# UNC-CFD/somar

Measured on AMD Instinct MI355X. Metric: pressure-Poisson V-cycles/sec, higher is better.
Workload: dtype f64; 1 GPU; C2 single-level 512^3 Poisson, diagonal stretched metric, Neumann, LevelGSRB V-cycle 2/2/2 + BiCGStab bottom; layout = 1 box(es) 512x512x512, one per GPU; mg_depth=8, cells=134217728

## Files before the change

somar_amd/build.py:

```python
import os
import subprocess
import sys

HERE = os.path.dirname(os.path.abspath(__file__))
CSRC = os.path.join(HERE, "csrc")
OUT = os.path.join(HERE, "libsomar_amd.so")
SOURCES = ["kernels.hip", "box_bicgstab.hip", "gsrb_fused.hip", "resid_march.hip", "multi_march.hip", "full19.hip", "full19_march.hip", "full19_fused.hip", "projection.hip", "line_gsrb.hip", "amr_kernels.hip", "leptic_kernels.hip", "maps.hip", "metric_refresh.hip", "box_io.hip", "tuning.cpp", "level.cpp", "solver.cpp", "solver_full.cpp", "solver_multi.cpp", "amr.cpp", "leptic.cpp", "comm_rccl.cpp", "comm_shm.cpp", "capi.cpp"]
HEADERS = ["common.h", "devbuf.h", "tuning.h", "kernels.h", "level.h", "march_plan.h", "stencil_point.h", "solver.h", "amr.h", "leptic.h", os.path.join("..", "..", "include", "somar_amd.h")]
HIPCC = os.environ.get("HIPCC", "/opt/rocm/bin/hipcc")
FLAGS = ["--offload-arch=gfx950", "-O3", "-std=c++17", "-fPIC", "-ffp-contract=off", "-fno-fast-math",
         "-Wall", "-Wno-unused-result", "-Wno-unused-value", "-I/opt/rocm/include"]


EXTRA = os.environ.get("SOMAR_EXTRA_FLAGS", "").split()


def _stale():
    if not os.path.exists(OUT):
        return True
    t = os.path.getmtime(OUT)
    return any(os.path.getmtime(os.path.join(CSRC, f)) > t for f in SOURCES + HEADERS)


def build(force=False, verbose=False):
    if not (force or _stale()):
        return OUT
    objs = []
    for f in SOURCES:
        src = os.path.join(CSRC, f)
        obj = os.path.join(CSRC, os.path.splitext(f)[0] + ".o")
        cmd = [HIPCC] + FLAGS + EXTRA + (["-x", "hip"] if f.endswith(".cpp") else []) + ["-c", src, "-o", obj]
        if verbose:
            print(" ".join(cmd))
        subprocess.check_call(cmd)
        objs.append(obj)
    cmd = [HIPCC, "--offload-arch=gfx950", "-shared", "-fPIC", "-o", OUT] + objs + ["-ldl", "-lrt"]
    if verbose:
        print(" ".join(cmd))
    subprocess.check_call(cmd)
    return OUT


if __name__ == "__main__":
    print(build(force="--force" in sys.argv, verbose=True))
```

somar_amd/csrc/kernels.h:

```cpp
#pragma once
#include "common.h"

namespace somar {

struct TileSpan {
    const Tile* p = nullptr;
    int n = 0;
    int classes = 0;
};

struct LevelDev {
    const Tile* tiles = nullptr;
    int ntiles = 0;
    int tile_j = 4;
    const CopyItem* tile_items = nullptr;
    const int* tile_item_start = nullptr;
    int ghost_gy = 16;
    const PatchDesc* patches = nullptr;
    int npatches = 0;
    double* jg[3] = {nullptr, nullptr, nullptr};
    double* jinv = nullptr;
    double* lapdiag = nullptr;
    double* jgf[3][3] = {{nullptr, nullptr, nullptr}, {nullptr, nullptr, nullptr}, {nullptr, nullptr, nullptr}};
    StencilParams P;
// ... 97 lines not shown
void launch_convert(hipStream_t st, float* dst, const double* src, long long n, double scale = 1.0);
void launch_incr2(hipStream_t st, double* y1, const double* x1, double a1, double* y2, const double* x2, double a2, long long n);
void launch_bicg_p(hipStream_t st, double* p, const double* v, const double* r, double beta, double bw, long long n);
void launch_incr_copy(hipStream_t st, double* y, double* x, double a, long long n);
void launch_scale(hipStream_t st, double* y, double a, long long n);
void launch_mul(hipStream_t st, double* y, const double* x, long long n);
void launch_axby(hipStream_t st, double* z, const double* x, const double* y, double a, double b, long long n);
struct ScalarPublish { double* host_dst; unsigned long long* host_seq; unsigned long long seq; };
struct TinyBicg {
    const Tile* tiles; int ntiles; int tile_j;
    const PatchDesc* patches; int npatches;
    const CopyItem* items; int nitems;
    long long field_elems;
    const double* jg[3]; const double* jinv; const double* lapd;
    StencilParams P;
    double* phi; const double* rhs;
    double* w[8];
    int imax, numRestarts, normType, precondIters;
    double eps, reps, hang, small, metric;
    double* info;
    ScalarPublish pub;
};
void launch_tiny_bicgstab(hipStream_t st, const LevelDev& L, const CopyItem* items, int nitems, long long field_elems, TinyBicg A);
constexpr int BOX_MAX_WG = 128, BOX_MAX_CELLS = 2048;
constexpr int BOX_FAB_MAX = 2048, BOX_MAX_ENT = 2048, BOX_MAX_STAGES = 63, BOX_MAX_NEUM = 512;
struct alignas(4) BoxProgEntry {
    unsigned short dst, s1, s2, s3;
    unsigned char kind, flags;
    unsigned short nslot;
};
struct BoxBicg {
    const PatchDesc* patches; int npatches;
    const int* nb; const int* cstart;
    const double* jg[3]; const double* jinv; const double* lapd;
    StencilParams P;
    double* phi; const double* rhs;
    double* z[2];
    int imax, numRestarts, normType, precondIters;
    double eps, reps, hang, small, metric;
    double* sums;
    unsigned* sync;
    int full;
    const double* jgf[3][3];
    const int* fab_src; const int* fab_start;
    const BoxProgEntry* ent[2]; const int* ent_first[2];
    const int* stg[2]; const int* stg_first[2];
    const int* nfg[2]; const int* nfg_first[2];
    long long* dbg;
    int serial;
    double* info;
    ScalarPublish pub;
};
void launch_box_bicgstab(hipStream_t st, const LevelDev& L, int max_box_cells, BoxBicg A);
void launch_stream_probe(hipStream_t st, int kind, int workgroups, double* const* in6, double* out, long long cells);
constexpr int MM_CH = 64;
struct CoarsenItem { const double* fine; double* crse; int patch; int dir; };
void launch_coarsen_metric(hipStream_t st, const LevelDev& C, const LevelDev& F, const CoarsenItem* items, int nitems,
                           int gy, const int r[3]);
struct MinMaxItem { const double* a; const PatchDesc* patches; int patch; int dir; };
void launch_minmax_all(hipStream_t st, const MinMaxItem* items, int nitems, double* out);
void launch_reduce(hipStream_t st, const LevelDev& L, const double* a, const double* b, int mode, double* partials,
                   double* out, bool ordered = false, const ScalarPublish* pub = nullptr);
void launch_reduce(hipStream_t st, const LevelDev& L, const float* a, const double* b, int mode, double* partials,
                   double* out);
void launch_ord_fill(hipStream_t st, const LevelDev& L, const long long* start, const double* a, const double* b,
                     int mode, double dxProduct, double* X, double* Y);
void launch_reduce_ordered_flat(hipStream_t st, int nboxes, const long long* box_start, const double* X, const double* Y,
                                int mode, double* out);
void launch_div_mac(hipStream_t st, const LevelDev& L, double* out, const double* u0, const double* u1,
                    const double* u2, double dt);
void launch_jgup_from_dxdxi(hipStream_t st, long long n, int mu, const double* const x9[9], const double* J, double scale,
                            double* out);
void launch_altered_jgup(hipStream_t st, long long n, double* dest, const double* nsq, const double* dmu,
                         const double* dnu, const double* ix, const double* jy, const double* iy, const double* jx,
                         const double* gup, const double* J, double theta, double coriolisF, bool offdiag);
void launch_face_axpy(hipStream_t st, const LevelDev& L, double* const vel[3], double* const grad[3], double s);
void launch_mac_correct(hipStream_t st, const LevelDev& L, double* const vel[3], const double* phi, double dtScale);
void launch_face_wall(hipStream_t st, const LevelDev& L, double* const edge[3]);
void launch_map_metric(hipStream_t st, const LevelDev& L, int kind, const double dXi[3], const double Lc[3],
                       const double* d_depth, const int dlo[2], const int dn[2], bool diagonal, const double* domLen = nullptr);
void launch_face_bc(hipStream_t st, const LevelDev& L, double* const edge[3], const int kind[6], const double value[6]);
void launch_cell_to_edge(hipStream_t st, const LevelDev& L, double* const edge[3], double* const cc[3], bool wall);
void launch_cc_correct(hipStream_t st, const LevelDev& L, double* const cc[3], const double* phi, double dtScale);
void launch_edge_to_cell_axpy(hipStream_t st, const LevelDev& L, double* const cc[3], double* const grad[3], double dtScale);
void launch_cf_homog(hipStream_t st, const CFCell* cells, int n, double* phi, const double c1[3], const double c2[3],
                     const double fac[3]);
void launch_copy_items2(hipStream_t st, const PatchDesc* spatches, const PatchDesc* dpatches, const CopyItem* items,
                        int nitems, const double* src, double* dst);
void launch_fill_hash(hipStream_t st, const LevelDev& L, double* f, unsigned long long seed);
constexpr int BIO_THREADS = 256, BIO_KC = 8;
struct BoxIoItem {
    int clo[3];
    int cpj;
    long long cpk;
    long long coff;
    int rlo[3];
    int n[3];
    int patch;
    int comp;
    int slot;
    int tile0, tiles_ij;
    int pad_;
};
void launch_box_io(hipStream_t st, const LevelDev& L, const BoxIoItem* items, double* const* ptrs, int nitems, int ntiles,
                   double* const field[3], bool to_level);

// ... 2 lines not shown
```

somar_amd/csrc/solver.cpp:

```cpp
#include "solver.h"

#include <array>
#include <chrono>
#include <cmath>
#include <cstdio>
#include <cstdlib>
#include <cstring>

namespace somar {

static const int S_MAX_COARSE = 4;
enum { SLOT_TMP = 0, SLOT_SUMS = 8, NSLOTS = 16 };

PressureSolver::PressureSolver(Comm* comm, hipStream_t shared, const Tuning& tune) : tune_(tune), comm_(comm ? comm : &self_)
{
    if (shared) { st_ = shared; own_stream_ = false; }
    else SOMAR_HIP(hipStreamCreateWithFlags(&st_, hipStreamNonBlocking));
    d_scalars = DevBuf<double>::zeros(NSLOTS);
    SOMAR_HIP(hipDeviceSynchronize());
    SOMAR_HIP(hipHostMalloc(&h_scalars, (NSLOTS + 2) * sizeof(double), hipHostMallocCoherent | hipHostMallocMapped));
    h_seq_ = reinterpret_cast<unsigned long long*>(h_scalars + NSLOTS);
    *h_seq_ = 0;
}

PressureSolver::~PressureSolver()
{
    drop_graphs();
    mp_free();
    mc_free();
    if (st_) hipStreamSynchronize(st_);
    if (st_comm_) { hipStreamSynchronize(st_comm_); hipStreamDestroy(st_comm_); }
    if (ev_ready_) hipEventDestroy(ev_ready_);
    if (ev_done_) hipEventDestroy(ev_done_);
    for (Prof& p : prof_) {
        for (hipEvent_t e : p.a) hipEventDestroy(e);
        for (hipEvent_t e : p.b) hipEventDestroy(e);
    }
    if (h_scalars) hipHostFree(h_scalars);
    coarse_.reset();
    lev.clear();
    if (st_ && own_stream_) hipStreamDestroy(st_);
}

void PressureSolver::sync() { SOMAR_HIP(hipStreamSynchronize(st_)); }

void PressureSolver::profile_enable(bool on)
{
    const int POOL = 4096;
    if (on)
        for (Prof& p : prof_) {
            while ((int)p.a.size() < POOL) {
                hipEvent_t e0, e1;
// ... 222 lines not shown
    std::unique_ptr<Level> C(new Level);
    C->active[2] = F.active[2];
    C->alpha = F.alpha;
    C->beta = F.beta;
    std::vector<IBox> cb;
    for (const IBox& b : F.boxes) cb.push_back(b.coarsen(r));
    double cdx[3];
    for (int d = 0; d < 3; ++d) cdx[d] = F.dx[d] * (double)r[d];
    C->define(F.domain.coarsen(r), F.periodic, cdx, F.bc_type, cb, F.owner, comm_, tune_);
    C->alloc_metric();
    if (hasCF_) C->define_cf(dxCrse_);
    for (int pi = 0; pi < C->npatches(); ++pi)
        for (int d = 0; d < nd; ++d)
            launch_avg_face(st_, C->dev, F.dev, pi, C->hpatches[pi].n, C->dev.jg[d], F.dev.jg[d], d, r);
    if (full_) {
        C->alloc_cross_metric();
        for (int pi = 0; pi < C->npatches(); ++pi)
            for (int d = 0; d < nd; ++d)
                for (int c = 0; c < nd; ++c)
                    if (c != d)
                        launch_avg_face(st_, C->dev, F.dev, pi, C->hpatches[pi].n, C->dev.jgf[d][c], F.dev.jgf[d][c], d, r);
    }
    launch_avg_harmonic(st_, C->dev, F.dev, C->dev.jinv, F.dev.jinv, r);
    launch_lapdiag(st_, C->dev);
    fill_metric_ghosts(*C);
    lev.push_back(std::move(C));
    return true;
}

void PressureSolver::fill_metric_ghosts(Level& L)
{
    for (int d = 0; d < 3; ++d)
        if (L.cf_faces[d]) L.cf_faces[d]->run(L.dev.jg[d], L.dev.jg[d], st_);
    for (int d = 0; d < 3; ++d) xchg(L, L.dev.jg[d]);
    if (full_)
        for (int d = 0; d < 3; ++d)
            for (int c = 0; c < 3; ++c)
                if (c != d && L.dev.jgf[d][c]) xchg(L, L.dev.jgf[d][c]);
    xchg(L, L.dev.jinv);
}

void PressureSolver::probe_null_space(int d)
{
    Level& L = *lev[d];
    DevBuf<double> phi = L.alloc_field(), rhs0 = L.alloc_field(), res = L.alloc_field();
    launch_set(st_, phi, L.field_elems, 0.0);
    apply_op(d, rhs0, phi);
    launch_set(st_, phi, L.field_elems, 1.0);
    residual(d, res, phi, rhs0);
    launch_reduce(st_, L.dev, res, nullptr, 3, d_partials, d_scalars + SLOT_TMP);
    comm_->allreduce(d_scalars + SLOT_TMP, 1, 1, st_);
    const double maxNorm = std::fabs(fetch_scalar(SLOT_TMP));
    L.zeroAvg = maxNorm < 0.01 * (probe_eps > 0.0 ? probe_eps : prm.eps);
}

void PressureSolver::finalize()
{
    SOMAR_CHECK(!lev.empty() && !finalized, "finalize before define / twice");
    if (mp_mode_ == 1) {
        const std::string why = mixed_refusal();
        SOMAR_CHECK(why.empty(), "finalize: mixed precision (set_precision mode 1) is not available for " + why);
    }
    const bool timing = tune_.timing != 0;
    auto now = [&]() { if (timing) hipDeviceSynchronize(); return std::chrono::steady_clock::now(); };
    auto secs = [](std::chrono::steady_clock::time_point a, std::chrono::steady_clock::time_point b) {
        return std::chrono::duration<double>(b - a).count();
    };
    const auto t0 = now();
    launch_lapdiag(st_, lev[0]->dev);
    fill_metric_ghosts(*lev[0]);
    int depth = 1;
    while (build_coarser(depth)) {
        if (comm_->size > 1 && lev[depth]->valid_cells_global <= tune_.agglom_cells && !full_) {
            build_agglomerated_tail(depth);
            break;
        }
        ++depth;
    }
    const auto t1 = now();
    detect_metric_flags();
    {
        const int min_box = (int)tune_.fused19_min_box;
        fused19_.assign(lev.size(), 0);
        for (size_t d = 0; d < lev.size(); ++d) {
            Level& L = *lev[d];
            bool ok = full_ && min_box >= 0 && full_march((int)d) && tune_.full_rows == 8 && !L.boxes.empty();
            for (const IBox& b : L.boxes)
                for (int a = 0; a < 3; ++a) ok = ok && b.size(a) >= std::max(min_box, 8) && (a != 0 || b.size(a) % 2 == 0);
            fused19_[d] = ok ? 1 : 0;
            if (ok != L.march.fused19) L.build_march_tiles(MarchRequest{L.march.narrow7, L.march.tall7, ok});
        }
    }
    choose_narrow_tiles();
    const auto t2 = now();
    struct Report {
        bool on; std::chrono::steady_clock::time_point t0, t1, t2; long long cells;
        ~Report() {
            if (!on) return;
            hipDeviceSynchronize();
            const auto t3 = std::chrono::steady_clock::now();
            fprintf(stderr, "[somar timing] finalize %lld cells: coarse hierarchy %.3f s, uniform detection %.3f s, fields + probes %.3f s\n",
                    cells, std::chrono::duration<double>(t1 - t0).count(), std::chrono::duration<double>(t2 - t1).count(),
                    std::chrono::duration<double>(t3 - t2).count());
        }
    } report{timing, t0, t1, t2, lev[0]->valid_cells_global};
    (void)secs;
// ... 1049 lines not shown
        double* eb[3] = {e[0], e[1], prm.spaceDim == 3 ? e[2] : nullptr};
        launch_face_bc(st_, lev[0]->dev, eb, velbc_kind_, velbc_value_);
    }
    divergence_mac(out, dt);
}

void PressureSolver::cc_correct(double* phi, double dt)
{
    Level& L = *lev[0];
    xchg(L, phi);
    double* c[3] = {cc_vel(0), cc_vel(1), prm.spaceDim == 3 ? cc_vel(2) : nullptr};
    const double dtScale = dt == 0.0 ? -1.0 : -dt;
    if (full_) {
        mac_grad_full(phi);
        launch_edge_to_cell_axpy(st_, L.dev, c, f_flux, dtScale);
        return;
    }
    launch_cc_correct(st_, L.dev, c, phi, dtScale);
}

void PressureSolver::cc_project(double dt, bool zeroPressure, bool forceHomogeneous, bool wall, SolveStats& s)
{
    check_idle("cc_project");
    divergence_cc(f_rhs, dt, wall);
    solve(zeroPressure, forceHomogeneous, s);
    cc_correct(f_phi, dt);
    sync();
}

void PressureSolver::fill_hash(int d, double* f, unsigned long long seed)
{
    launch_fill_hash(st_, lev[d]->dev, f, seed);
}

void PressureSolver::vcycle(double* e, const double* res, bool e_zero)
{
    check_idle("vcycle");
    if (mp_K_ > 0) {
        double rnorm = norm(0, res, 0);
        if (!e_zero) rnorm = std::max(rnorm, norm(0, e, 0));
        vcycle_mixed(e, res, rnorm, e_zero, false);
        return;
    }
    cycle(0, e, res, e_zero);
}

void PressureSolver::cycle_bottom_relax(double* corr, const double* res, bool corr_zero)
{
    const int d = (int)lev.size() - 1;
    if (lev[d]->domain.numPts() == 1) {
        relax(d, corr, res, 1, corr_zero);
        return;
    }
    if (corr_zero && prm.num_smooth_bottom == 0) launch_set(st_, corr, lev[d]->field_elems, 0.0);
    relax(d, corr, res, prm.num_smooth_bottom, corr_zero && prm.num_smooth_bottom > 0);
}

void PressureSolver::cycle_down(int d, double* corr, const double* res, bool corr_zero)
{
    if (corr_zero && prm.num_smooth_down == 0) launch_set(st_, corr, lev[d]->field_elems, 0.0);
    relax(d, corr, res, prm.num_smooth_down, corr_zero && prm.num_smooth_down > 0);
    restrict_residual(d, f_res[d + 1], corr, res);
}

void PressureSolver::cycle_up(int d, double* corr, const double* res)
{
    if (fold_prolong(d)) {
        fold_up(d, corr, res, f_corr[d + 1].get(), true);
        return;
    }
    const double* shift = prolong_increment(d, corr, f_corr[d + 1], fused_relax(d, prm.num_smooth_up));
    relax(d, corr, res, prm.num_smooth_up, false, shift);
}

void PressureSolver::cycle(int d, double* corr, const double* res, bool corr_zero)
{
    if (coarse_ && d == agglom_depth_) {
        agglom_cycle(corr, res, corr_zero);
        return;
    }
    const int D = (int)lev.size();
    if (mini_depth_ > 0 && d == mini_depth_ - 1) {
        (void)corr_zero;
        launch_set(st_, corr, lev[d]->field_elems, 0.0);
        return;
    }
    if (d == D - 1) {
        cycle_bottom_relax(corr, res, corr_zero);
        if (lev[d]->domain.numPts() != 1) bottom_solve(corr, res);
        return;
    }
    const int ncyc = cycle_override_ ? cycle_override_ : prm.numMG;
    SOMAR_CHECK(ncyc != 0, "numMG must not be 0");
    if (ncyc < 0) {
        const int cycles = -ncyc;
        Level& L = *lev[d];
        if (corr_zero) launch_set(st_, corr, L.field_elems, 0.0);
        restrict_residual(d, f_res[d + 1], corr, res);
        cycle(d + 1, f_corr[d + 1], f_res[d + 1], true);
        prolong_increment(d, corr, f_corr[d + 1]);
        relax(d, corr, res, prm.num_smooth_down);
        for (int img = 0; img < cycles; ++img) {
            restrict_residual(d, f_res[d + 1], corr, res);
            const int saved = cycle_override_;
            cycle_override_ = 1;
            try {
                cycle(d + 1, f_corr[d + 1], f_res[d + 1], true);
            } catch (...) {
                cycle_override_ = saved;
                throw;
            }
            cycle_override_ = saved;
            prolong_increment(d, corr, f_corr[d + 1]);
        }
        relax(d, corr, res, prm.num_smooth_up);
        return;
    }
    if (mini_depth_ == 0 && graph_cycle(d, corr, res, corr_zero)) return;
    cycle_down(d, corr, res, corr_zero);
// ... 820 lines not shown
```

somar_amd/csrc/solver.h:

```cpp
#pragma once
#include <exception>
#include <memory>
#include <vector>

#include "level.h"

namespace somar {

enum { RELAX_JACOBI = 0, RELAX_LEVEL_GSRB = 1, RELAX_LOOSE_GSRB = 2, RELAX_LINE_GSRB = 3 };
enum { PRECOND_NONE = -1, PRECOND_DIAG_RELAX = 0, PRECOND_DIAG_LINE_RELAX = 1 };

struct SolverParams {
    int imin = 5, imax = 20;
    double eps = 1e-6, hang = 1e-15, normThresh = 1e-30;
    int num_smooth_down = 2, num_smooth_up = 2, num_smooth_bottom = 2, num_smooth_precond = 2;
    int numMG = 1, maxDepth = -1, precondMode = PRECOND_DIAG_RELAX, relaxMode = RELAX_LEVEL_GSRB;
    int verbosity = 0;
    int spaceDim = 3;
    int bottom_imax = 80, bottom_numRestarts = 5, bottom_normType = 2, bottom_verbosity = 0;
    double bottom_eps = 1e-6, bottom_reps = 1e-12, bottom_hang = 1e-15, bottom_small = 1e-30;
};

struct SolveStats {
    int iters = 0;
// ... 372 lines not shown
        double alpha0 = 0.0, beta0 = 1.0;
        OpState st;
        ~CompOp() { drop_graph(st.cg); }
    };
    double ab_scale_[2] = {1.0, 1.0};
    int op_in_place_ = 0;
    CompOp* comp_op(int comp) const { return comp > 0 && comp <= (int)comps_.size() ? comps_[comp - 1].op.get() : nullptr; }
    void exchange_op(OpState& o);
    template <class Fn>
    void on_op(int comp, Fn f)
    {
        CompOp* o = comp_op(comp);
        if (!o) { f(); return; }
        exchange_op(o->st);
        op_in_place_ = comp;
        try { f(); } catch (...) { exchange_op(o->st); op_in_place_ = 0; throw; }
        exchange_op(o->st);
        op_in_place_ = 0;
    }
    bool probe_op(CompOp& o, int* depth);
    void ensure_face_copiers(const int bc[3][2]);
    StencilParams comp_params(int comp, int d) const;
    LevelDev comp_level(int comp, int d) const;
    void comp_diri(int comp, int d, double* phi, bool homogeneous);
    template <int NF>
    bool field_ops(int d, const int* comp, FieldOps<NF>& O);
    template <int NF>
    void sweep_launch(int d, const int* comp, const SweepFields<NF>& S, int mode);
    template <int NF>
    void resid_launch(int d, const int* comp, const ResidFields<NF>& R, bool restrict);
    std::vector<GhostOp> make_diri_ops(int d, const int bc[3][2], const double val[3][2], bool sides_of_solver) const;
    int graph_from_ = -1;
    bool capturing_ = false;
    bool diri_ = false;
    double bc_value_[3][2] = {{0, 0}, {0, 0}, {0, 0}};
    std::vector<DevBuf<GhostOp>> d_diri_ops_;
    std::vector<int> n_diri_ops_;
    DevBuf<GhostOp> d_extrapbc_ops_;
    int n_extrapbc_ops_ = 0;
    void build_diri_ops(int d);
    void apply_diri(int d, double* phi, bool homogeneous);
    bool face_[3][2] = {{false, false}, {false, false}, {false, false}};
    std::vector<double> face_plane_[3][2];
    std::vector<long long> face_off_;
    std::vector<double> h_bcface_;
    DevBuf<double> d_bcface_;
    std::vector<GhostOp> h_diri_ops0_;
    void build_face_slices();
    void fill_face_values();
    void set_diri_op(GhostOp& op) const;
    void refresh_diri_ops();
    int mini_depth_ = 0;
    int cycle_override_ = 0;
    void cycle_down(int d, double* corr, const double* res, bool corr_zero);
    void cycle_up(int d, double* corr, const double* res);
    void cycle_bottom_relax(double* corr, const double* res, bool corr_zero);
    bool graph_cycle(int d, double* corr, const double* res, bool corr_zero);
    void drop_graphs();
    struct Prof { std::vector<hipEvent_t> a, b; int used = 0; };
    Prof prof_[4];
    template <class T>
    void xchg(const Level& L, T* f);
    hipStream_t st_comm_ = nullptr;
    hipEvent_t ev_ready_ = nullptr, ev_done_ = nullptr;
    bool resid_overlap(const Level& L) const
    {
        return !tune_.no_overlap && !L.plan.peers.empty() && !L.rtiles.own.empty() && !capturing_ && !profiling_ && !diri_;
    }
    template <class T, class Run>
    void overlapped(const Level& L, T* f, const SplitTileTable& table, Run run)
    {
        if (!st_comm_) {
            SOMAR_HIP(hipStreamCreateWithFlags(&st_comm_, hipStreamNonBlocking));
            SOMAR_HIP(hipEventCreateWithFlags(&ev_ready_, hipEventDisableTiming));
            SOMAR_HIP(hipEventCreateWithFlags(&ev_done_, hipEventDisableTiming));
        }
        SOMAR_HIP(hipEventRecord(ev_ready_, st_));
        SOMAR_HIP(hipStreamWaitEvent(st_comm_, ev_ready_, 0));
        L.exchange_local(f, st_);
        run(table.own.span());
        L.exchange_remote(f, st_comm_);
        SOMAR_HIP(hipEventRecord(ev_done_, st_comm_));
        SOMAR_HIP(hipStreamWaitEvent(st_, ev_done_, 0));
        run(table.rem.span());
        ++counters[0];
    }
    bool fused_overlap(const Level& L) const
    {
        return !tune_.no_overlap && !L.plan.peers.empty() && !L.ftiles.own.empty() && !capturing_ && !profiling_;
    }
    bool profiling_ = false;
    void prof_begin(int k);
    void prof_end(int k);
    struct ProfScope {
        PressureSolver* s;
        int k, unwinding;
        ProfScope(PressureSolver& ps, int d, int k_, bool on = true)
            : s(ps.profiling_ && d == 0 && on ? &ps : nullptr), k(k_), unwinding(std::uncaught_exceptions())
        {
            if (s) s->prof_begin(k);
        }
        ~ProfScope() noexcept(false) { if (s && std::uncaught_exceptions() == unwinding) s->prof_end(k); }
        ProfScope(const ProfScope&) = delete;
    };
};

// ... 2 lines not shown
```

somar_amd/csrc/solver_multi.cpp:

```cpp
#include "solver.h"

#include <cmath>

namespace somar {

std::string PressureSolver::multi_refusal() const
{
    if (amr_member_) return "a level of an AMR hierarchy (the composite cycle carries one field)";
    if (full_) return "a non-diagonal metric (19-point operator)";
    if (prm.relaxMode != RELAX_LEVEL_GSRB) return "a relax_mode other than LevelGSRB";
    if (prm.numMG != 1) return "num_mg != 1 (W- and F-cycles run plain passes, no folding)";
    if (hasCF_ || !forcedRatios.empty()) return "a level with coarse-fine boundaries";
    if (comm_->size > 1 || coarse_) return "a level sharded over more than one rank";
    if (mp_mode_ == 1) return "set_precision mode 1 (the fp32 cycle carries one field)";
    return "";
}

void PressureSolver::set_components(int ncomp, long long min_cells)
{
    check_idle("set_components");
    SOMAR_CHECK(ncomp >= 1 && ncomp <= MC_MAX, "set_components: 1 to 4 components");
    if (ncomp > 1) {
        const std::string why = multi_refusal();
        SOMAR_CHECK(why.empty(), "set_components: more than one component is not available for " + why);
// ... 67 lines not shown
        SOMAR_CHECK(f.classes == 0 && r.classes == 0, "internal: the N-field kernels take class-0 tiles");
        for (const Tile& t : r.tiles) SOMAR_CHECK(!(t.j0 & 1) && !(t.k0 & 1), "internal: restriction tiles start on even rows and planes");
        mc_ftiles_[d].assign(std::move(f.tiles), 0);
        mc_rtiles_[d].assign(std::move(r.tiles), 0);
    }
    mc_K_ = K;
    sync();
}

void PressureSolver::swap_comp(int comp)
{
    if (comp == 0) return;
    Component& c = comps_.at(comp - 1);
    std::swap(f_phi, c.phi);
    std::swap(f_rhs, c.rhs);
    std::swap(f_uberRes, c.res);
    std::swap(f_uberCorr, c.corr);
    std::swap(f_best, c.best);
    for (int q = 0; q < 3; ++q) std::swap(f_heat[q], c.heat[q]);
    if (c.op) {
        exchange_op(c.op->st);
        op_in_place_ = op_in_place_ == comp ? 0 : comp;
    }
}

void PressureSolver::exchange_op(OpState& o)
{
    const Level& L0 = *lev[0];
    OpState live;
    for (int a = 0; a < 3; ++a)
        for (int s = 0; s < 2; ++s) { live.bc[a][s] = L0.bc_type[a][s]; live.val[a][s] = bc_value_[a][s]; bc_value_[a][s] = o.val[a][s]; }
    live.alpha = L0.alpha;
    live.beta = L0.beta;
    for (size_t d = 0; d < lev.size(); ++d) {
        Level& L = *lev[d];
        for (int a = 0; a < 3; ++a)
            for (int s = 0; s < 2; ++s) L.bc_type[a][s] = o.bc[a][s];
        L.alpha = o.alpha;
        L.beta = o.beta;
        const char z = L.zeroAvg ? 1 : 0;
        L.zeroAvg = o.zeroAvg[d] != 0;
        o.zeroAvg[d] = z;
        L.refresh_params();
    }
    for (int a = 0; a < 3; ++a)
        for (int s = 0; s < 2; ++s) { o.bc[a][s] = live.bc[a][s]; o.val[a][s] = live.val[a][s]; }
    o.alpha = live.alpha;
    o.beta = live.beta;
    std::swap(o.diri, diri_);
    o.d_ops.swap(d_diri_ops_);
    o.n_ops.swap(n_diri_ops_);
    o.h_ops0.swap(h_diri_ops0_);
    std::swap(o.cg, cg_);
}

bool PressureSolver::probe_op(CompOp& o, int* depth)
{
    const double a = o.st.alpha, b = o.st.beta;
    o.st.alpha = o.alpha0;
    o.st.beta = o.beta0;
    exchange_op(o.st);
    bool any = false;
    try {
        for (int d = 0; d < (int)lev.size(); ++d) {
            probe_null_space(d);
            if (lev[d]->zeroAvg && !any) { any = true; if (depth) *depth = d; }
        }
    } catch (...) {
        exchange_op(o.st);
        o.st.alpha = a;
        o.st.beta = b;
        throw;
    }
    exchange_op(o.st);
    o.st.alpha = a;
    o.st.beta = b;
    return any;
}

void PressureSolver::ensure_face_copiers(const int bc[3][2])
{
    for (auto& Lp : lev) {
        Level& L = *Lp;
        for (int a = 0; a < 3; ++a) {
            if (!L.active[a] || L.periodic[a] || bc[a][1] != BC_DIRI || L.cf_faces[a]) continue;
            int gh[3];
            for (int e = 0; e < 3; ++e) gh[e] = L.active[e] ? FRAME : 0;
            L.cf_faces[a].reset(new Copier);
            L.cf_faces[a]->define_faces(L.domain, L.periodic, L, a, gh, comm_);
            SOMAR_HIP(hipDeviceSynchronize());
            L.cf_faces[a]->run(L.dev.jg[a], L.dev.jg[a], st_);
            xchg(L, L.dev.jg[a]);
        }
    }
}

void PressureSolver::comp_set_op(int comp, const int bc6[6], const double val6[6], double alpha, double beta)
{
    check_idle("comp_set_op");
    SOMAR_CHECK(finalized && ncomp_ > 1, "comp_set_op: after set_components has accepted more than one component");
    SOMAR_CHECK(comp != 0, "comp_set_op: component 0 is the solver's create-time operator and is not settable");
    SOMAR_CHECK(comp > 0 && comp < ncomp_, "comp_set_op: component out of range (1 .. ncomp - 1)");
    SOMAR_CHECK(bc6 && val6, "comp_set_op: null argument");
    SOMAR_CHECK(op_in_place_ == 0, "internal: comp_set_op while a component's operator is in place");
    const Level& L0 = *lev[0];
    std::unique_ptr<CompOp> n(new CompOp);
// ... 498 lines not shown
```

Baseline: 104.0 V-cycles/s.

## Fuse small multigrid levels into single-workgroup LDS-resident down/up leg kernels

Adds single-workgroup kernels that run an entire V-cycle leg on coarse levels of up to 4096 cells. The down leg does relax, residual and restriction, and the up leg does prolongation, optional zero-average removal and relax. The field stays in shared memory, replacing many tiny launches per coarse level. Eligibility is computed per depth so that only single-box, 7-point, single-rank, non-Dirichlet levels take the path. The cost is that only one workgroup works on these levels, and the fused kernels duplicate the boundary-handling logic of the existing path.

```diff
diff --git a/somar_amd/build.py b/somar_amd/build.py
--- a/somar_amd/build.py
+++ b/somar_amd/build.py
@@ -5,8 +5,8 @@
 HERE = os.path.dirname(os.path.abspath(__file__))
 CSRC = os.path.join(HERE, "csrc")
 OUT = os.path.join(HERE, "libsomar_amd.so")
-SOURCES = ["kernels.hip", "box_bicgstab.hip", "gsrb_fused.hip", "resid_march.hip", "multi_march.hip", "full19.hip", "full19_march.hip", "full19_fused.hip", "projection.hip", "line_gsrb.hip", "amr_kernels.hip", "leptic_kernels.hip", "maps.hip", "metric_refresh.hip", "box_io.hip", "tuning.cpp", "level.cpp", "solver.cpp", "solver_full.cpp", "solver_multi.cpp", "amr.cpp", "leptic.cpp", "comm_rccl.cpp", "comm_shm.cpp", "capi.cpp"]
-HEADERS = ["common.h", "devbuf.h", "tuning.h", "kernels.h", "level.h", "march_plan.h", "stencil_point.h", "solver.h", "amr.h", "leptic.h", os.path.join("..", "..", "include", "somar_amd.h")]
+SOURCES = ["kernels.hip", "box_bicgstab.hip", "level_legs.hip", "gsrb_fused.hip", "resid_march.hip", "multi_march.hip", "full19.hip", "full19_march.hip", "full19_fused.hip", "projection.hip", "line_gsrb.hip", "amr_kernels.hip", "leptic_kernels.hip", "maps.hip", "metric_refresh.hip", "box_io.hip", "tuning.cpp", "level.cpp", "solver.cpp", "solver_full.cpp", "solver_multi.cpp", "amr.cpp", "leptic.cpp", "comm_rccl.cpp", "comm_shm.cpp", "capi.cpp"]
+HEADERS = ["common.h", "devbuf.h", "tuning.h", "kernels.h", "level.h", "march_plan.h", "leg_plan.h", "stencil_point.h", "solver.h", "amr.h", "leptic.h", os.path.join("..", "..", "include", "somar_amd.h")]
 HIPCC = os.environ.get("HIPCC", "/opt/rocm/bin/hipcc")
 FLAGS = ["--offload-arch=gfx950", "-O3", "-std=c++17", "-fPIC", "-ffp-contract=off", "-fno-fast-math",
          "-Wall", "-Wno-unused-result", "-Wno-unused-value", "-I/opt/rocm/include"]
diff --git a/somar_amd/csrc/kernels.h b/somar_amd/csrc/kernels.h
--- a/somar_amd/csrc/kernels.h
+++ b/somar_amd/csrc/kernels.h
@@ -173,6 +173,21 @@
     ScalarPublish pub;
 };
 void launch_box_bicgstab(hipStream_t st, const LevelDev& L, int max_box_cells, BoxBicg A);
+constexpr int LEG_MAX_CELLS = 4096;
+struct LegArgs {
+    const PatchDesc* patches;
+    const double* jg[3]; const double* jinv; const double* lapd;
+    StencilParams P;
+    const PatchDesc* cpatches;
+    double* corr; const double* res;
+    double* cres;
+    const double* ccorr;
+    int r[3];
+    int sweeps;
+    int corr_zero;
+    int zero_avg; double dxProduct;
+};
+void launch_level_leg(hipStream_t st, const LevelDev& L, int box_cells, bool up, LegArgs A);
 void launch_stream_probe(hipStream_t st, int kind, int workgroups, double* const* in6, double* out, long long cells);
 constexpr int MM_CH = 64;
 struct CoarsenItem { const double* fine; double* crse; int patch; int dir; };
diff --git a/somar_amd/csrc/leg_plan.h b/somar_amd/csrc/leg_plan.h
--- /dev/null
+++ b/somar_amd/csrc/leg_plan.h
@@ -0,0 +1,74 @@
+#pragma once
+
+namespace somar {
+namespace leg_plan {
+
+struct Box {
+    int lo[3], hi[3];
+    int size(int a) const { return hi[a] - lo[a] + 1; }
+    long long cells() const { return (long long)size(0) * size(1) * size(2); }
+    bool same(const Box& o) const
+    {
+        for (int a = 0; a < 3; ++a)
+            if (lo[a] != o.lo[a] || hi[a] != o.hi[a]) return false;
+        return true;
+    }
+};
+
+struct Depth {
+    int nboxes = 0;
+    Box box{};
+    Box domain{};
+    int active[3] = {1, 1, 1};
+    int periodic[3] = {0, 0, 0};
+    int diri_sides = 0;
+    int cf_cells = 0;
+    int peers = 0;
+    bool zero_avg = false;
+    bool ordered = false;
+};
+
+struct Solver {
+    bool seven_point = true;
+    bool level_gsrb = true;
+    int ranks = 1;
+    bool box_bottom = true;
+    int max_cells = 0;
+};
+
+inline bool one_box(const Depth& L) { return L.nboxes == 1 && L.box.same(L.domain); }
+
+inline bool depth_ok(const Solver& S, const Depth& L)
+{
+    if (!S.box_bottom || !S.seven_point || !S.level_gsrb || S.ranks != 1) return false;
+    if (!one_box(L) || L.box.cells() < 1 || L.box.cells() > S.max_cells) return false;
+    if (!(L.active[0] && L.active[1] && L.active[2])) return false;
+    if (L.diri_sides != 0 || L.cf_cells != 0 || L.peers != 0) return false;
+    if (L.zero_avg && !L.ordered) return false;
+    for (int a = 0; a < 3; ++a)
+        if (L.periodic[a] && L.box.size(a) > 1 && (L.box.size(a) & 1)) return false;
+    return true;
+}
+
+inline bool leg_eligible(const Solver& S, const Depth& L, const Depth* coarse, const int ratio[3])
+{
+    if (!depth_ok(S, L)) return false;
+    if (!coarse) return true;
+    if (!one_box(*coarse)) return false;
+    for (int a = 0; a < 3; ++a) {
+        const int r = ratio[a];
+        if (r != 1 && r != 2) return false;
+        if (coarse->domain.lo[a] * r != L.domain.lo[a] || (coarse->domain.hi[a] + 1) * r != L.domain.hi[a] + 1) return false;
+    }
+    return true;
+}
+
+inline int cells_per_thread(int cells) { return cells <= 512 ? 1 : cells <= 1024 ? 2 : 4; }
+inline int threads(int cells)
+{
+    const int per = cells_per_thread(cells), want = (cells + per - 1) / per;
+    return (want + 63) / 64 * 64;
+}
+
+}
+}
diff --git a/somar_amd/csrc/level_legs.hip b/somar_amd/csrc/level_legs.hip
--- /dev/null
+++ b/somar_amd/csrc/level_legs.hip
@@ -0,0 +1,364 @@
+#include "common.h"
+#include "kernels.h"
+#include "leg_plan.h"
+
+namespace somar {
+
+namespace {
+__device__ __forceinline__ long long cidx(const PatchDesc& p, int i, int j, int k)
+{
+    return p.off + i + (long long)p.pj * j + p.pk * k;
+}
+
+constexpr unsigned LEG_ACT = 0x4000u, LEG_BLACK = 0x8000u;
+template <int CPT, bool LDSC>
+struct LegCells {
+    unsigned flg[CPT];
+    double jl[CPT][3], jh[CPT][3];
+    double rJi[LDSC ? 1 : CPT], rdg[LDSC ? 1 : CPT], rrhs[LDSC ? 1 : CPT];
+    double *QJ, *QD, *QR;
+    __device__ __forceinline__ bool act(int q) const { return (flg[q] & LEG_ACT) != 0; }
+    __device__ __forceinline__ unsigned flags(int q) const
+    {
+        unsigned f = flg[q];
+        if constexpr (LDSC) asm volatile("" : "+v"(f));
+        return f;
+    }
+    __device__ __forceinline__ double Ji(int q, int idx) const { if constexpr (LDSC) return QJ[idx]; else return rJi[q]; }
+    __device__ __forceinline__ double dg(int q, int idx) const { if constexpr (LDSC) return QD[idx]; else return rdg[q]; }
+    __device__ __forceinline__ double rhs(int q, int idx) const { if constexpr (LDSC) return QR[idx]; else return rrhs[q]; }
+    int n0, n01, cells;
+    int wrap[3];
+    double xxScale, yyScale, zzScale, sx, sy, sz, alpha, beta;
+
+    __device__ __forceinline__ long long offset(const PatchDesc& p, int idx) const
+    {
+        const int li = idx % p.n[0], r = idx / p.n[0];
+        return cidx(p, li, r % p.n[1], r / p.n[1]);
+    }
+    __device__ __forceinline__ void setup(const LegArgs& A, const PatchDesc& p, int tid, int nth, double* qj, double* qd, double* qr)
+    {
+        const StencilParams& P = A.P;
+        QJ = qj; QD = qd; QR = qr;
+        n0 = p.n[0];
+        n01 = p.n[0] * p.n[1];
+        cells = n01 * p.n[2];
+        const int cst[3] = {1, n0, n01};
+        for (int a = 0; a < 3; ++a) wrap[a] = P.periodic[a] ? (p.n[a] - 1) * cst[a] : 0;
+        xxScale = 1.0 / (P.dx[0] * P.dx[0]); yyScale = 1.0 / (P.dx[1] * P.dx[1]); zzScale = 1.0 / (P.dx[2] * P.dx[2]);
+        sx = 1.0 / P.dx[0]; sy = 1.0 / P.dx[1]; sz = 1.0 / P.dx[2];
+        alpha = P.alpha; beta = P.beta;
+#pragma unroll
+        for (int q = 0; q < CPT; ++q) {
+            const int idx = cell(q, tid, nth);
+            const bool have = idx < cells;
+            const int ii = have ? idx : 0;
+            const int li = ii % p.n[0], r = ii / p.n[0];
+            const int lj = r % p.n[1], lk = r / p.n[1];
+            const long long cc = cidx(p, li, lj, lk);
+            const int gi = p.lo[0] + li, gj = p.lo[1] + lj, gk = p.lo[2] + lk;
+            jl[q][0] = A.jg[0][cc]; jh[q][0] = A.jg[0][cc + 1];
+            jl[q][1] = A.jg[1][cc]; jh[q][1] = A.jg[1][cc + p.pj];
+            jl[q][2] = A.jg[2][cc]; jh[q][2] = A.jg[2][cc + p.pk];
+            const double Jc = A.jinv[cc];
+            const double dd = alpha + beta * A.lapd[cc];
+            const bool xl = gi == P.dom_lo[0], xh = gi == P.dom_hi[0], yl = gj == P.dom_lo[1], yh = gj == P.dom_hi[1];
+            const bool zl = gk == P.dom_lo[2], zh = gk == P.dom_hi[2];
+            const bool onb = xl || xh || yl || yh || zl || zh;
+            const bool nxl = xl && P.neum[0][0], nxh = xh && P.neum[0][1], nyl = yl && P.neum[1][0], nyh = yh && P.neum[1][1];
+            const bool nzl = zl && P.neum[2][0], nzh = zh && P.neum[2][1];
+            flg[q] = (nxl ? 1u : 0u) | (nxh ? 2u : 0u) | (nyl ? 4u : 0u) | (nyh ? 8u : 0u) | (nzl ? 16u : 0u) | (nzh ? 32u : 0u) |
+                     (onb ? 64u : 0u) | (li == 0 ? 0x100u : 0u) | (li == p.n[0] - 1 ? 0x200u : 0u) | (lj == 0 ? 0x400u : 0u) |
+                     (lj == p.n[1] - 1 ? 0x800u : 0u) | (lk == 0 ? 0x1000u : 0u) | (lk == p.n[2] - 1 ? 0x2000u : 0u) |
+                     (have ? LEG_ACT : 0u) | (((gi + gj + gk) & 1) ? LEG_BLACK : 0u);
+            double dgc;
+            if (!onb) {
+                dgc = dd;
+            } else {
+                double ld = 0.0;
+                if (!nxl) ld = ld - xxScale * jl[q][0];
+                if (!nyl) ld = ld - yyScale * jl[q][1];
+                if (!nzl) ld = ld - zzScale * jl[q][2];
+                if (!nxh) ld = ld - xxScale * jh[q][0];
+                if (!nyh) ld = ld - yyScale * jh[q][1];
+                if (!nzh) ld = ld - zzScale * jh[q][2];
+                ld = ld * Jc;
+                dgc = alpha + beta * ld;
+            }
+            if constexpr (LDSC) {
+                if (have) { QJ[idx] = Jc; QD[idx] = dgc; QR[idx] = A.res[cc]; }
+            } else {
+                rJi[q] = Jc; rdg[q] = dgc; rrhs[q] = A.res[cc];
+            }
+            if constexpr (LDSC) __builtin_amdgcn_sched_barrier(0);
+        }
+    }
+    __device__ __forceinline__ void gather(const double* Z, int idx, unsigned f, double v[6]) const
+    {
+        v[0] = Z[(f & 0x100u) ? idx + wrap[0] : idx - 1];
+        v[1] = Z[(f & 0x200u) ? idx - wrap[0] : idx + 1];
+        v[2] = Z[(f & 0x400u) ? idx + wrap[1] : idx - n0];
+        v[3] = Z[(f & 0x800u) ? idx - wrap[1] : idx + n0];
+        v[4] = Z[(f & 0x1000u) ? idx + wrap[2] : idx - n01];
+        v[5] = Z[(f & 0x2000u) ? idx - wrap[2] : idx + n01];
+    }
+    __device__ __forceinline__ double relax_vals(const double* Z, int idx, unsigned f0, const double l[3], const double h[3], double Jiv,
+                                                 double dgv, double rhsv) const
+    {
+        double v[6];
+        unsigned f = f0;
+        if constexpr (LDSC) asm volatile("" : "+v"(f));
+        gather(Z, idx, f, v);
+        double lphi;
+        if (!(f & 64u)) {
+            const double JDxx = xxScale * (h[0] * v[1] + l[0] * v[0]);
+            const double JDyy = yyScale * (h[1] * v[3] + l[1] * v[2]);
+            const double JDzz = zzScale * (h[2] * v[5] + l[2] * v[4]);
+            lphi = beta * Jiv * (JDxx + JDyy + JDzz);
+        } else {
+            double JDloX = 0, JDhiX = 0, JDloY = 0, JDhiY = 0, JDloZ = 0, JDhiZ = 0;
+            if (!(f & 1u)) JDloX = l[0] * v[0];
+            if (!(f & 4u)) JDloY = l[1] * v[2];
+            if (!(f & 16u)) JDloZ = l[2] * v[4];
+            if (!(f & 2u)) JDhiX = h[0] * v[1];
+            if (!(f & 8u)) JDhiY = h[1] * v[3];
+            if (!(f & 32u)) JDhiZ = h[2] * v[5];
+            lphi = beta * Jiv * ((JDloX + JDhiX) * xxScale + (JDloY + JDhiY) * yyScale + (JDloZ + JDhiZ) * zzScale);
+        }
+        return (rhsv - lphi) / dgv;
+    }
+    __device__ __forceinline__ double relax_cell(int q, const double* Z, int idx) const
+    {
+        return relax_vals(Z, idx, flg[q], jl[q], jh[q], Ji(q, idx), dg(q, idx), rhs(q, idx));
+    }
+    __device__ __forceinline__ double op_cell(int q, const double* Z, int idx, double pc) const
+    {
+        double v[6];
+        const unsigned f = flags(q);
+        gather(Z, idx, f, v);
+        double fxl = jl[q][0] * sx * (pc - v[0]);
+        double fxh = jh[q][0] * sx * (v[1] - pc);
+        double fyl = jl[q][1] * sy * (pc - v[2]);
+        double fyh = jh[q][1] * sy * (v[3] - pc);
+        double fzl = jl[q][2] * sz * (pc - v[4]);
+        double fzh = jh[q][2] * sz * (v[5] - pc);
+        if (f & 1u) fxl = 0.0;
+        if (f & 2u) fxh = 0.0;
+        if (f & 4u) fyl = 0.0;
+        if (f & 8u) fyh = 0.0;
+        if (f & 16u) fzl = 0.0;
+        if (f & 32u) fzh = 0.0;
+        fxl *= beta; fxh *= beta; fyl *= beta; fyh *= beta; fzl *= beta; fzh *= beta;
+        double l = Ji(q, idx) * ((fxh - fxl) * sx + (fyh - fyl) * sy + (fzh - fzl) * sz);
+        if (alpha != 0.0) l = alpha * pc + 1.0 * l;
+        return l;
+    }
+    static __device__ __forceinline__ int cell(int q, int tid, int nth)
+    {
+        if constexpr (CPT == 1) return tid;
+        else return 2 * tid + (q & 1) + (q >> 1) * 2 * nth;
+    }
+    __device__ __forceinline__ void sweeps(int n, double* Z, double* phv, int tid, int nth) const
+    {
+        for (int it = 0; it < n; ++it)
+            for (int pass = 0; pass < 2; ++pass) {
+                const unsigned want = LEG_ACT | (pass ? LEG_BLACK : 0u);
+                if constexpr (CPT == 1) {
+                    if ((flg[0] & (LEG_ACT | LEG_BLACK)) == want) {
+                        phv[0] = relax_cell(0, Z, tid);
+                        Z[tid] = phv[0];
+                    }
+                } else {
+#pragma unroll
+                    for (int m = 0; m < CPT; m += 2) {
+                        const bool a0 = (flg[m] & (LEG_ACT | LEG_BLACK)) == want, a1 = (flg[m + 1] & (LEG_ACT | LEG_BLACK)) == want;
+                        if (a0 || a1) {
+                            int pick = a0 ? 0 : 1;
+                            asm volatile("" : "+v"(pick));
+                            const bool second = pick != 0;
+                            const int idx = cell(m, tid, nth) + (second ? 1 : 0);
+                            double l[3], h[3];
+#pragma unroll
+                            for (int a = 0; a < 3; ++a) { l[a] = second ? jl[m + 1][a] : jl[m][a]; h[a] = second ? jh[m + 1][a] : jh[m][a]; }
+                            const double Jiv = LDSC ? QJ[idx] : (second ? rJi[LDSC ? 0 : m + 1] : rJi[LDSC ? 0 : m]);
+                            const double dgv = LDSC ? QD[idx] : (second ? rdg[LDSC ? 0 : m + 1] : rdg[LDSC ? 0 : m]);
+                            const double rhsv = LDSC ? QR[idx] : (second ? rrhs[LDSC ? 0 : m + 1] : rrhs[LDSC ? 0 : m]);
+                            const double out = relax_vals(Z, idx, second ? flg[m + 1] : flg[m], l, h, Jiv, dgv, rhsv);
+                            if (second) phv[m + 1] = out; else phv[m] = out;
+                            Z[idx] = out;
+                        }
+                        if (a0 && a1) {
+                            phv[m + 1] = relax_cell(m + 1, Z, cell(m + 1, tid, nth));
+                            Z[cell(m + 1, tid, nth)] = phv[m + 1];
+                        }
+                        if constexpr (LDSC) __builtin_amdgcn_sched_barrier(0);
+                    }
+                }
+                __syncthreads();
+            }
+    }
+};
+}
+
+template <int CPT, int MAXT>
+__global__ __launch_bounds__(MAXT) void k_leg_down(LegArgs A)
+{
+    constexpr bool LDSC = CPT == 4;
+    __shared__ double Z[LEG_MAX_CELLS], W[LEG_MAX_CELLS];
+    __shared__ double D[LDSC ? LEG_MAX_CELLS : 1], R[LDSC ? LEG_MAX_CELLS : 1];
+    const int tid = threadIdx.x, nth = blockDim.x;
+    const PatchDesc p = A.patches[0];
+    LegCells<CPT, LDSC> T;
+    T.setup(A, p, tid, nth, W, D, R);
+    double phv[CPT];
+#pragma unroll
+    for (int q = 0; q < CPT; ++q) {
+        const int idx = T.cell(q, tid, nth);
+        phv[q] = (T.act(q) && !A.corr_zero) ? A.corr[T.offset(p, idx)] : 0.0;
+        if (T.act(q)) {
+            Z[idx] = phv[q];
+            if constexpr (!LDSC) W[idx] = T.rJi[q];
+        }
+    }
+    __syncthreads();
+    T.sweeps(A.sweeps, Z, phv, tid, nth);
+#pragma unroll
+    for (int q = 0; q < CPT; ++q) if (T.act(q)) A.corr[T.offset(p, T.cell(q, tid, nth))] = phv[q];
+    if (!A.cpatches) return;
+    const double* RES = LDSC ? R : Z;
+    if constexpr (LDSC) {
+#pragma unroll
+        for (int q = 0; q < CPT; ++q) {
+            const int idx = T.cell(q, tid, nth);
+            if (T.act(q)) R[idx] = R[idx] - T.op_cell(q, Z, idx, phv[q]);
+            __builtin_amdgcn_sched_barrier(0);
+        }
+    } else {
+        double rv[CPT];
+#pragma unroll
+        for (int q = 0; q < CPT; ++q) {
+            const int idx = T.cell(q, tid, nth);
+            rv[q] = T.act(q) ? T.rhs(q, idx) - T.op_cell(q, Z, idx, phv[q]) : 0.0;
+        }
+        __syncthreads();
+#pragma unroll
+        for (int q = 0; q < CPT; ++q) if (T.act(q)) Z[T.cell(q, tid, nth)] = rv[q];
+    }
+    __syncthreads();
+    const PatchDesc cp = A.cpatches[0];
+    const int r0 = A.r[0], r1 = A.r[1], r2 = A.r[2];
+    const int ccells = cp.n[0] * cp.n[1] * cp.n[2];
+    for (int ci = tid; ci < ccells; ci += nth) {
+        const int li = ci % cp.n[0], r = ci / cp.n[0];
+        const int lj = r % cp.n[1], lk = r / cp.n[1];
+        double s = 0.0, sj = 0.0;
+        for (int ii2 = 0; ii2 < r2; ++ii2)
+            for (int ii1 = 0; ii1 < r1; ++ii1)
+                for (int ii0 = 0; ii0 < r0; ++ii0) {
+                    const int f = (li * r0 + ii0) + T.n0 * (lj * r1 + ii1) + T.n01 * (lk * r2 + ii2);
+                    const double ji = W[f];
+                    s = s + RES[f] / ji;
+                    sj = sj + 1.0 / ji;
+                }
+        A.cres[cidx(cp, li, lj, lk)] = s / sj;
+    }
+}
+
+template <int CPT, int MAXT>
+__global__ __launch_bounds__(MAXT) void k_leg_up(LegArgs A)
+{
+    constexpr bool LDSC = CPT == 4;
+    __shared__ double Z[LEG_MAX_CELLS], W[LEG_MAX_CELLS];
+    __shared__ double D[LDSC ? LEG_MAX_CELLS : 1], R[LDSC ? LEG_MAX_CELLS : 1];
+    __shared__ double S[2];
+    const int tid = threadIdx.x, nth = blockDim.x;
+    const PatchDesc p = A.patches[0];
+    const PatchDesc cp = A.cpatches[0];
+    const int cells = p.n[0] * p.n[1] * p.n[2];
+    double phv[CPT];
+#pragma unroll
+    for (int q = 0; q < CPT; ++q) {
+        const int idx = LegCells<CPT, LDSC>::cell(q, tid, nth);
+        const bool have = idx < cells;
+        const int ii = have ? idx : 0;
+        const int li = ii % p.n[0], r = ii / p.n[0];
+        const int lj = r % p.n[1], lk = r / p.n[1];
+        const long long cc = cidx(p, li, lj, lk);
+        phv[q] = have ? A.corr[cc] + A.ccorr[cidx(cp, li / A.r[0], lj / A.r[1], lk / A.r[2])] : 0.0;
+        if (A.zero_avg && have) {
+            const double y = A.dxProduct / A.jinv[cc];
+            W[idx] = y;
+            Z[idx] = y * phv[q];
+        }
+    }
+    if (A.zero_avg) {
+        __syncthreads();
+        auto chain = [&](const double* X) {
+            constexpr int B = 16;
+            double run = 0.0;
+            double xa[B], xb[B];
+            auto fetch = [&](double* x, int q0) {
+#pragma unroll
+                for (int j = 0; j < B; ++j) x[j] = X[q0 + j];
+            };
+            auto add = [&](const double* x) {
+#pragma unroll
+                for (int j = 0; j < B; ++j) run = run + x[j];
+            };
+            const int nb = cells / B;
+            int b = 0;
+            if (nb > 0) fetch(xa, 0);
+            for (; b + 2 <= nb; b += 2) {
+                fetch(xb, (b + 1) * B);
+                add(xa);
+                fetch(xa, (b + 2 < nb ? b + 2 : 0) * B);
+                add(xb);
+            }
+            if (b < nb) add(xa);
+            for (int q = nb * B; q < cells; ++q) run = run + X[q];
+            return run;
+        };
+        const int wave = tid >> 6, vwave = nth > 64 ? 1 : 0;
+        if (wave == 0) {
+            const double r = chain(Z);
+            if (tid == 0) S[0] = r;
+        }
+        if (wave == vwave) {
+            const double r = chain(W);
+            if ((tid & 63) == 0) S[1] = r;
+        }
+        __syncthreads();
+        const double avg = S[0] / S[1];
+#pragma unroll
+        for (int q = 0; q < CPT; ++q) phv[q] -= avg;
+    }
+    LegCells<CPT, LDSC> T;
+    T.setup(A, p, tid, nth, W, D, R);
+#pragma unroll
+    for (int q = 0; q < CPT; ++q) if (T.act(q)) Z[T.cell(q, tid, nth)] = phv[q];
+    __syncthreads();
+    T.sweeps(A.sweeps, Z, phv, tid, nth);
+#pragma unroll
+    for (int q = 0; q < CPT; ++q) if (T.act(q)) A.corr[T.offset(p, T.cell(q, tid, nth))] = phv[q];
+}
+
+void launch_level_leg(hipStream_t st, const LevelDev& L, int box_cells, bool up, LegArgs A)
+{
+    SOMAR_CHECK(L.npatches == 1 && box_cells >= 1 && box_cells <= LEG_MAX_CELLS, "level leg: level outside the kernel's limits");
+    SOMAR_CHECK(!up || (A.cpatches && A.ccorr), "level leg: the up leg needs the coarser depth");
+    A.patches = L.patches;
+    for (int d = 0; d < 3; ++d) A.jg[d] = L.jg[d];
+    A.jinv = L.jinv; A.lapd = L.lapdiag; A.P = L.P;
+    const int cpt = leg_plan::cells_per_thread(box_cells), nth = leg_plan::threads(box_cells);
+    if (up) {
+        if (cpt == 1) hipLaunchKernelGGL((k_leg_up<1, 512>), dim3(1), dim3(nth), 0, st, A);
+        else if (cpt == 2) hipLaunchKernelGGL((k_leg_up<2, 512>), dim3(1), dim3(nth), 0, st, A);
+        else hipLaunchKernelGGL((k_leg_up<4, 1024>), dim3(1), dim3(nth), 0, st, A);
+    } else {
+        if (cpt == 1) hipLaunchKernelGGL((k_leg_down<1, 512>), dim3(1), dim3(nth), 0, st, A);
+        else if (cpt == 2) hipLaunchKernelGGL((k_leg_down<2, 512>), dim3(1), dim3(nth), 0, st, A);
+        else hipLaunchKernelGGL((k_leg_down<4, 1024>), dim3(1), dim3(nth), 0, st, A);
+    }
+}
+
+}
diff --git a/somar_amd/csrc/solver.cpp b/somar_amd/csrc/solver.cpp
--- a/somar_amd/csrc/solver.cpp
+++ b/somar_amd/csrc/solver.cpp
@@ -1,3 +1,4 @@
+#include "leg_plan.h"
 #include "solver.h"
 
 #include <array>
@@ -326,6 +327,67 @@
     comm_->allreduce(d_scalars + SLOT_TMP, 1, 1, st_);
     const double maxNorm = std::fabs(fetch_scalar(SLOT_TMP));
     L.zeroAvg = maxNorm < 0.01 * (probe_eps > 0.0 ? probe_eps : prm.eps);
+    update_leg(d);
+}
+
+void PressureSolver::update_leg(int d)
+{
+    if (leg_.size() != lev.size()) leg_.assign(lev.size(), 0);
+    namespace lp = leg_plan;
+    auto facts = [&](int q) {
+        const Level& L = *lev[q];
+        lp::Depth F;
+        F.nboxes = (int)L.boxes.size();
+        for (int a = 0; a < 3; ++a) {
+            if (!L.boxes.empty()) { F.box.lo[a] = L.boxes[0].lo[a]; F.box.hi[a] = L.boxes[0].hi[a]; }
+            F.domain.lo[a] = L.domain.lo[a];
+            F.domain.hi[a] = L.domain.hi[a];
+            F.active[a] = L.active[a];
+            F.periodic[a] = L.periodic[a] ? 1 : 0;
+            for (int s = 0; s < 2; ++s)
+                if (!L.periodic[a] && L.bc_type[a][s] == BC_DIRI) ++F.diri_sides;
+        }
+        if (diri_) F.diri_sides = std::max(F.diri_sides, 1);
+        F.cf_cells = L.ncf;
+        F.peers = (int)L.plan.peers.size();
+        F.zero_avg = L.zeroAvg;
+        F.ordered = ordered(q);
+        return F;
+    };
+    lp::Solver S;
+    S.seven_point = !full_;
+    S.level_gsrb = prm.relaxMode == RELAX_LEVEL_GSRB;
+    S.ranks = comm_->size;
+    S.box_bottom = tune_.box_bottom != 0;
+    S.max_cells = LEG_MAX_CELLS;
+    const lp::Depth F = facts(d);
+    bool ok;
+    if (d + 1 < (int)lev.size()) {
+        const lp::Depth C = facts(d + 1);
+        ok = lp::leg_eligible(S, F, &C, lev[d]->mgCrseRefRatio);
+    } else {
+        ok = !coarse_ && lev[d]->domain.numPts() != 1 && lp::leg_eligible(S, F, nullptr, lev[d]->mgCrseRefRatio);
+    }
+    ok = ok && lev[d]->npatches() == 1 && lev[d]->field_elems <= 0x7fffffffll;
+    leg_[d] = ok ? 1 : 0;
+}
+
+void PressureSolver::run_leg(int d, bool up, double* corr, const double* res, int sweeps, bool corr_zero)
+{
+    Level& L = *lev[d];
+    const bool bottom = d + 1 >= (int)lev.size();
+    LegArgs A{};
+    A.cpatches = bottom ? nullptr : lev[d + 1]->dev.patches;
+    A.corr = corr;
+    A.res = res;
+    A.cres = (bottom || up) ? nullptr : f_res[d + 1].get();
+    A.ccorr = up ? f_corr[d + 1].get() : nullptr;
+    for (int a = 0; a < 3; ++a) A.r[a] = L.mgCrseRefRatio[a];
+    A.sweeps = unswept(d) ? 0 : sweeps;
+    A.corr_zero = corr_zero ? 1 : 0;
+    A.zero_avg = up && L.zeroAvg ? 1 : 0;
+    A.dxProduct = L.dxProduct;
+    launch_level_leg(st_, L.dev, (int)L.valid_cells_global, up, A);
 }
 
 void PressureSolver::finalize()
@@ -1481,12 +1543,20 @@
         relax(d, corr, res, 1, corr_zero);
         return;
     }
+    if (leg(d)) {
+        run_leg(d, false, corr, res, prm.num_smooth_bottom, corr_zero);
+        return;
+    }
     if (corr_zero && prm.num_smooth_bottom == 0) launch_set(st_, corr, lev[d]->field_elems, 0.0);
     relax(d, corr, res, prm.num_smooth_bottom, corr_zero && prm.num_smooth_bottom > 0);
 }
 
 void PressureSolver::cycle_down(int d, double* corr, const double* res, bool corr_zero)
 {
+    if (leg(d)) {
+        run_leg(d, false, corr, res, prm.num_smooth_down, corr_zero);
+        return;
+    }
     if (corr_zero && prm.num_smooth_down == 0) launch_set(st_, corr, lev[d]->field_elems, 0.0);
     relax(d, corr, res, prm.num_smooth_down, corr_zero && prm.num_smooth_down > 0);
     restrict_residual(d, f_res[d + 1], corr, res);
@@ -1494,6 +1564,10 @@
 
 void PressureSolver::cycle_up(int d, double* corr, const double* res)
 {
+    if (leg(d)) {
+        run_leg(d, true, corr, res, prm.num_smooth_up, false);
+        return;
+    }
     if (fold_prolong(d)) {
         fold_up(d, corr, res, f_corr[d + 1].get(), true);
         return;
diff --git a/somar_amd/csrc/solver.h b/somar_amd/csrc/solver.h
--- a/somar_amd/csrc/solver.h
+++ b/somar_amd/csrc/solver.h
@@ -448,6 +448,10 @@
     void refresh_diri_ops();
     int mini_depth_ = 0;
     int cycle_override_ = 0;
+    std::vector<char> leg_;
+    bool leg(int d) const { return d < (int)leg_.size() && leg_[d] != 0; }
+    void update_leg(int d);
+    void run_leg(int d, bool up, double* corr, const double* res, int sweeps, bool corr_zero);
     void cycle_down(int d, double* corr, const double* res, bool corr_zero);
     void cycle_up(int d, double* corr, const double* res);
     void cycle_bottom_relax(double* corr, const double* res, bool corr_zero);
diff --git a/somar_amd/csrc/solver_multi.cpp b/somar_amd/csrc/solver_multi.cpp
--- a/somar_amd/csrc/solver_multi.cpp
+++ b/somar_amd/csrc/solver_multi.cpp
@@ -143,6 +143,7 @@
     o.n_ops.swap(n_diri_ops_);
     o.h_ops0.swap(h_diri_ops0_);
     std::swap(o.cg, cg_);
+    for (int d = 0; d < (int)lev.size(); ++d) update_leg(d);
 }
 
 bool PressureSolver::probe_op(CompOp& o, int* depth)
```

Result: no change. 104.7 V-cycles/s (median of 6 runs) (+0.7%).
